# AnyDSL/rodent

Measured on AMD Instinct MI355X. Metric: Mrays/s, higher is better.
Workload: dtype f32; 1 GPU; atrium.bvh + atrium-primary.rays (1024x1024 primary rays, tmax 5000, closest hit); bvh_layout=BVH2, kernel=k_bvh2_top_auto<false,15, 255, 16, 32>, variant=top, parallelism=replicated BVH x 1, world_size=1

## Files before the change

### include/rodent_traversal.h

```cpp
#ifndef RODENT_TRAVERSAL_H
#define RODENT_TRAVERSAL_H

#include <stdint.h>
#include <stddef.h>

#ifdef __cplusplus
extern "C" {
#endif


struct Node2 {
    float   bounds[12];
    int32_t child[2];
    int32_t pad[2];
};

struct Tri1 {
    float   v0[3];  int32_t pad;
    float   e1[3];  int32_t geom_id;
    float   e2[3];  int32_t prim_id;
};

struct Node4 {
    float   bounds[6][4];
// ... 35 lines not shown
        const struct Ray1* rays, struct Hit1* hits, int32_t num_rays);
void hip_occluded_single_ray1_bvh4_tri4(int32_t dev,
        const struct Node4* nodes, const struct Tri4* tris,
        const struct Ray1* rays, struct Hit1* hits, int32_t num_rays);
void hip_intersect_single_ray1_bvh8_tri4(int32_t dev,
        const struct Node8* nodes, const struct Tri4* tris,
        const struct Ray1* rays, struct Hit1* hits, int32_t num_rays);
void hip_occluded_single_ray1_bvh8_tri4(int32_t dev,
        const struct Node8* nodes, const struct Tri4* tris,
        const struct Ray1* rays, struct Hit1* hits, int32_t num_rays);

void hip_traverse_bvh2_tri1_async(int32_t dev,
        const struct Node2* nodes, const struct Tri1* tris,
        const struct Ray1* rays, struct Hit1* hits, int32_t num_rays,
        int32_t any_hit, int32_t variant, void* stream);
void hip_traverse_bvh4_tri4_async(int32_t dev,
        const struct Node4* nodes, const struct Tri4* tris,
        const struct Ray1* rays, struct Hit1* hits, int32_t num_rays,
        int32_t any_hit, int32_t variant, void* stream);
void hip_traverse_bvh8_tri4_async(int32_t dev,
        const struct Node8* nodes, const struct Tri4* tris,
        const struct Ray1* rays, struct Hit1* hits, int32_t num_rays,
        int32_t any_hit, int32_t variant, void* stream);
int32_t rodent_hip_check_errors(int32_t dev, void* stream);

uint64_t    rodent_hip_get_kernel_time(void);
int32_t     rodent_hip_device_count(void);
int32_t     rodent_hip_num_variants(int32_t bvh_width);
void        rodent_hip_phased_min_rays(int32_t rays);
void        rodent_hip_top_min_rays(int32_t rays);
void        rodent_hip_schedule_history(int32_t enable);
void        rodent_hip_ray_kind_hint(int32_t enable);
void        rodent_hip_ray_grid(int32_t width);
int32_t     rodent_hip_is_lab_build(void);
const char* rodent_hip_variant_name(int32_t bvh_width, int32_t variant);
const char* rodent_hip_kernel_name(int32_t bvh_width, int32_t variant, int32_t any_hit);
const char* rodent_hip_version(void);
const char* rodent_hip_source_digest(void);
void        rodent_hip_read_stats(int32_t dev, uint64_t* out8);
void        rodent_hip_read_trace(int32_t dev, uint64_t* out);
void        rodent_hip_debug_set_perm(int32_t dev, const int32_t* device_perm);

#ifdef __cplusplus
}
#endif
#endif
```

### rodent_amd/abi.py

```python
from __future__ import annotations

import ctypes as C
import os
from pathlib import Path

import numpy as np
import torch

from . import formats as F

LAB = os.environ.get("RODENT_HIP_LAB", "0") not in ("", "0")
LIB_PATH = Path(__file__).resolve().parent / "lib" / ("librodent_hip_lab.so" if LAB else "librodent_hip.so")
if os.environ.get("RODENT_HIP_LIB"):
    LIB_PATH = Path(os.environ["RODENT_HIP_LIB"]).resolve()

SYNC_ENTRY_POINTS = [
    "amdgpu_intersect_single_ray1_bvh2_tri1", "amdgpu_occluded_single_ray1_bvh2_tri1",
    "hip_intersect_single_ray1_bvh4_tri4", "hip_occluded_single_ray1_bvh4_tri4",
    "hip_intersect_single_ray1_bvh8_tri4", "hip_occluded_single_ray1_bvh8_tri4",
]
ASYNC_ENTRY_POINTS = ["hip_traverse_bvh2_tri1_async", "hip_traverse_bvh4_tri4_async", "hip_traverse_bvh8_tri4_async"]
EXPORTS = SYNC_ENTRY_POINTS + ASYNC_ENTRY_POINTS + [
    "rodent_hip_check_errors", "rodent_hip_get_kernel_time", "rodent_hip_device_count", "rodent_hip_num_variants",
        "rodent_hip_variant_name",
    "rodent_hip_kernel_name", "rodent_hip_version", "rodent_hip_source_digest", "rodent_hip_is_lab_build", "rodent_hip_phased_min_rays",
        "rodent_hip_top_min_rays", "rodent_hip_ray_kind_hint", "rodent_hip_ray_grid", "rodent_hip_schedule_history",
        "rodent_hip_read_stats", "rodent_hip_read_trace", "rodent_hip_debug_set_perm",
    "rodent_hip_build_scratch_bytes", "rodent_hip_build_bvh2_tri1", "rodent_hip_build_bvh2_tri1_sync",
    "rodent_hip_build_opt_scratch_bytes", "rodent_hip_build_bvh2_tri1_opt", "rodent_hip_build_bvh2_tri1_opt_sync",
    "rodent_hip_build_split_max_refs", "rodent_hip_build_split_scratch_bytes", "rodent_hip_build_bvh2_tri1_split",
    "rodent_hip_build_bvh2_tri1_split_sync",
    "rodent_hip_refit_scratch_bytes", "rodent_hip_refit_bvh2_tri1", "rodent_hip_refit_bvh2_tri1_sync",
    "rodent_hip_refit_wide_scratch_bytes", "rodent_hip_refit_bvh4_tri4", "rodent_hip_refit_bvh4_tri4_sync",
    "rodent_hip_refit_bvh8_tri4", "rodent_hip_refit_bvh8_tri4_sync",
]
BLOCK_OF_WIDTH = {2: F.BVH2_TRI1, 4: F.BVH4_TRI4, 8: F.BVH8_TRI4}

_lib = None


class BuildOptions(C.Structure):
    _fields_ = [("max_leaf", C.c_int32), ("treelet_passes", C.c_int32), ("node_cost", C.c_float), ("tri_cost", C.c_float)]


class SplitOptions(C.Structure):
    _fields_ = [("budget", C.c_float), ("max_pieces", C.c_int32)]


class MissingExtension(RuntimeError):
    pass


def lib():
    global _lib
    if _lib is None:
        if not LIB_PATH.exists():
            raise MissingExtension(f"{LIB_PATH} not built: run `python -m rodent_amd.build` (needs hipcc)")
        l = C.CDLL(str(LIB_PATH))
        vp, i32 = C.c_void_p, C.c_int32
        for name in SYNC_ENTRY_POINTS:
            fn = getattr(l, name); fn.restype = None; fn.argtypes = [i32, vp, vp, vp, vp, i32]
        for name in ASYNC_ENTRY_POINTS:
            fn = getattr(l, name); fn.restype = None; fn.argtypes = [i32, vp, vp, vp, vp, i32, i32, i32, vp]
        l.rodent_hip_check_errors.restype = i32; l.rodent_hip_check_errors.argtypes = [i32, vp]
        l.rodent_hip_is_lab_build.restype = i32; l.rodent_hip_is_lab_build.argtypes = []
        l.rodent_hip_phased_min_rays.restype = None; l.rodent_hip_phased_min_rays.argtypes = [i32]
        l.rodent_hip_top_min_rays.restype = None; l.rodent_hip_top_min_rays.argtypes = [i32]
        l.rodent_hip_get_kernel_time.restype = C.c_uint64; l.rodent_hip_get_kernel_time.argtypes = []
        l.rodent_hip_ray_kind_hint.restype = None; l.rodent_hip_ray_kind_hint.argtypes = [i32]
        l.rodent_hip_ray_grid.restype = None; l.rodent_hip_ray_grid.argtypes = [i32]
        l.rodent_hip_schedule_history.restype = None; l.rodent_hip_schedule_history.argtypes = [i32]
        l.rodent_hip_device_count.restype = i32; l.rodent_hip_device_count.argtypes = []
        l.rodent_hip_num_variants.restype = i32; l.rodent_hip_num_variants.argtypes = [i32]
        l.rodent_hip_variant_name.restype = C.c_char_p; l.rodent_hip_variant_name.argtypes = [i32, i32]
        l.rodent_hip_kernel_name.restype = C.c_char_p; l.rodent_hip_kernel_name.argtypes = [i32, i32, i32]
        l.rodent_hip_version.restype = C.c_char_p; l.rodent_hip_version.argtypes = []
        l.rodent_hip_source_digest.restype = C.c_char_p; l.rodent_hip_source_digest.argtypes = []
        l.rodent_hip_read_trace.restype = None; l.rodent_hip_read_trace.argtypes = [i32, C.c_void_p]
        l.rodent_hip_debug_set_perm.restype = None; l.rodent_hip_debug_set_perm.argtypes = [i32, C.c_void_p]
        l.rodent_hip_read_stats.restype = None; l.rodent_hip_read_stats.argtypes = [i32, C.POINTER(C.c_uint64)]
        l.rodent_hip_build_scratch_bytes.restype = C.c_int64; l.rodent_hip_build_scratch_bytes.argtypes = [i32]
        l.rodent_hip_build_bvh2_tri1.restype = i32
        l.rodent_hip_build_bvh2_tri1.argtypes = [i32, vp, i32, vp, i32, i32, vp, vp, vp, vp, vp]
        l.rodent_hip_build_bvh2_tri1_sync.restype = i32
        l.rodent_hip_build_bvh2_tri1_sync.argtypes = [i32, vp, i32, vp, i32, i32, vp, vp, C.POINTER(i32)]
        opt = C.POINTER(BuildOptions)
        l.rodent_hip_build_opt_scratch_bytes.restype = C.c_int64; l.rodent_hip_build_opt_scratch_bytes.argtypes = [i32, opt]
        l.rodent_hip_build_bvh2_tri1_opt.restype = i32
        l.rodent_hip_build_bvh2_tri1_opt.argtypes = [i32, vp, i32, vp, i32, opt, vp, vp, vp, vp, vp]
        l.rodent_hip_build_bvh2_tri1_opt_sync.restype = i32
        l.rodent_hip_build_bvh2_tri1_opt_sync.argtypes = [i32, vp, i32, vp, i32, opt, vp, vp, C.POINTER(i32)]
        spl = C.POINTER(SplitOptions)
        l.rodent_hip_build_split_max_refs.restype = C.c_int64; l.rodent_hip_build_split_max_refs.argtypes = [i32, spl]
        l.rodent_hip_build_split_scratch_bytes.restype = C.c_int64
        l.rodent_hip_build_split_scratch_bytes.argtypes = [i32, opt, spl]
        l.rodent_hip_build_bvh2_tri1_split.restype = i32
        l.rodent_hip_build_bvh2_tri1_split.argtypes = [i32, vp, i32, vp, i32, opt, spl, vp, vp, vp, vp, vp]
        l.rodent_hip_build_bvh2_tri1_split_sync.restype = i32
        l.rodent_hip_build_bvh2_tri1_split_sync.argtypes = [i32, vp, i32, vp, i32, opt, spl, vp, vp, C.POINTER(i32)]
        l.rodent_hip_refit_scratch_bytes.restype = C.c_int64; l.rodent_hip_refit_scratch_bytes.argtypes = [i32, i32]
        l.rodent_hip_refit_bvh2_tri1.restype = i32
        l.rodent_hip_refit_bvh2_tri1.argtypes = [i32, vp, i32, vp, i32, vp, i32, vp, i32, vp, vp, vp]
        l.rodent_hip_refit_bvh2_tri1_sync.restype = i32
# ... 84 lines not shown
    n = len(rays)
    rays_dev = to_device(rays, bvh.dev)
    hits_dev = torch.zeros(max(n, 1) * F.HIT1.itemsize, dtype=torch.uint8, device=f"cuda:{bvh.dev}")
    if variant is None:
        torch.cuda.synchronize(bvh.dev)
        name = {(2, False): "amdgpu_intersect_single_ray1_bvh2_tri1", (2, True): "amdgpu_occluded_single_ray1_bvh2_tri1",
                (4, False): "hip_intersect_single_ray1_bvh4_tri4", (4, True): "hip_occluded_single_ray1_bvh4_tri4",
                (8, False): "hip_intersect_single_ray1_bvh8_tri4",
                    (8, True): "hip_occluded_single_ray1_bvh8_tri4"}[(bvh.width, bool(any_hit))]
        getattr(lib(), name)(bvh.dev, bvh.nodes.data_ptr(), bvh.tris.data_ptr(), rays_dev.data_ptr(), hits_dev.data_ptr(), n)
    else:
        traverse_async(bvh, rays_dev, hits_dev, n, any_hit, variant)
        torch.cuda.synchronize(bvh.dev)
        check_errors(bvh.dev)
    return from_device(hits_dev, F.HIT1)[:n]


def schedule_history(enable: bool):
    lib().rodent_hip_schedule_history(int(bool(enable)))


def top_min_rays(rays: int):
    lib().rodent_hip_top_min_rays(int(rays))


def ray_kind_hint(enable: bool):
    lib().rodent_hip_ray_kind_hint(int(bool(enable)))


def ray_grid(width: int = -1):
    lib().rodent_hip_ray_grid(int(width))


def check_errors(dev=0, stream=None):
    import torch
    if stream is None:
        stream = torch.cuda.current_stream(dev)
    if lib().rodent_hip_check_errors(dev, C.c_void_p(stream.cuda_stream)):
        raise RuntimeError("rodent_hip: traversal stack overflow (more than 64 entries)")


def read_stats(dev=0):
    buf = (C.c_uint64 * 8)()
    lib().rodent_hip_read_stats(dev, buf)
    return list(buf)


def read_trace(dev=0, arm_only=False):
    if arm_only:
        lib().rodent_hip_read_trace(dev, None)
        return None
    buf = np.zeros((16384, 4), np.uint64)
    lib().rodent_hip_read_trace(dev, buf.ctypes.data_as(C.c_void_p))
    return buf
```

### rodent_amd/csrc/traversal.hip

```cpp
#include <hip/hip_runtime.h>

#include <algorithm>
#include <atomic>
#include <cstdint>
#include <cstdio>
#include <cstdlib>
#include <memory>
#include <mutex>
#include <utility>
#include <vector>

#include "device_buffer.h"
#include "rodent_traversal.h"
#include "traversal_device.h"

namespace {

using namespace rodent_dev;

template <bool ANY, bool WIDE = true>
__device__ __forceinline__ bool leaf_tri1(const Tri1* __restrict__ tris, int first, RayX& ray, HitAcc& hit) {
    int j = first;
    for (;;) {
        const float4* p = WIDE ? reinterpret_cast<const float4*>(tris + j)
// ... 83 lines not shown
        if (last) {
            ctl->stats[7] += (unsigned long long)count; ctl->counter = 0; ctl->deep_count = 0; ctl->finish_done = 0;
            report_error(ctl);
        }
    }
}

template <bool ANY>
__global__ __launch_bounds__(kWave) void k_bvh2_finish(const Node2* __restrict__ nodes, const Tri1* __restrict__ tris,
                                                        const Ray1* __restrict__ rays, Hit1* __restrict__ hits,
                                                        Ctl* ctl, const int* __restrict__ deep_list,
                                                            int* , int* phase_counters) {
    __shared__ int stack_lds[kStackCap * kWave];
    finish_launch<ANY>(nodes, tris, rays, hits, ctl, deep_list, (lds_int*)stack_lds, phase_counters, blockIdx.x, gridDim.x);
}

struct Lane {
    RayX ray;
    int top;
    lds_int* sp;
    int ray_id;
    bool found;
};
typedef const __attribute__((address_space(1))) char* gptr;
struct Bases { gptr node, tri; };
__device__ __forceinline__ Bases make_bases(const Node2* nodes, const Tri1* tris) {
    unsigned long long node_bits = reinterpret_cast<unsigned long long>(nodes - 1), tri_bits = reinterpret_cast<unsigned long long>(tris);
    asm volatile("" : "+v"(node_bits), "+v"(tri_bits));
    return Bases{(gptr)node_bits, (gptr)tri_bits};
}

typedef __attribute__((address_space(3))) float lds_float;
template <bool ANY, bool PF = false, bool TOP = false, bool LAZY = false, bool FENCE = false, bool SHARED = false, int SPILL = 0,
    int WPG = 1>
__device__ __forceinline__ void bvh2_step(Lane& L, const Bases& base, Hit1* __restrict__ hits, lds_int* sp_limit, Ctl* ctl,
    int* __restrict__ deep_list,
                                          bool prefetch = false, lds_int* pf_row = nullptr, lds_int* image = nullptr,
                                              lds_float* shared_tmax = nullptr,
                                          int* __restrict__ spill = nullptr) {
    const bool is_node = L.top > 0;
    typedef float f32x4 __attribute__((ext_vector_type(4)));
    typedef int i32x2 __attribute__((ext_vector_type(2)));
    f32x4 q0, q1, q2;
    i32x2 ch;
    int popped;
    float shared_now = 0.0f;
    if constexpr (TOP && !SHARED) {
        const unsigned idx = (unsigned)(is_node ? L.top : ~L.top), stride = is_node ? (unsigned)sizeof(Node2) : (unsigned)sizeof(Tri1);
        const gptr addr = (is_node ? base.node : base.tri) + (size_t)idx * stride;
        joint_fetch(q0, q1, q2, ch, popped, L.top >= kLdsTag, (unsigned)(size_t)image + (unsigned)(L.top - kLdsTag), addr,
            addr + (is_node ? 48u : 40u), L.sp);
    } else {
        if (TOP && L.top >= kLdsTag) {
            typedef __attribute__((address_space(3))) const char* lds_bytes;
            const lds_bytes rec = (lds_bytes)image + (unsigned)(L.top - kLdsTag);
            const __attribute__((address_space(3))) f32x4* p = (const __attribute__((address_space(3))) f32x4*)rec;
            q0 = p[0]; q1 = p[1]; q2 = p[2];
            ch = *(const __attribute__((address_space(3))) i32x2*)(rec + 48);
        } else {
            const unsigned idx = (unsigned)(is_node ? L.top : ~L.top), stride = is_node ? (unsigned)sizeof(Node2) : (unsigned)sizeof(Tri1);
            const gptr addr = (is_node ? base.node : base.tri) + (size_t)idx * stride;
            const __attribute__((address_space(1))) f32x4* p = (const __attribute__((address_space(1))) f32x4*)addr;
            q0 = p[0]; q1 = p[1]; q2 = p[2];
            ch = *(const __attribute__((address_space(1))) i32x2*)(addr + (is_node ? 48u : 40u));
        }
        popped = *L.sp;
        if (SHARED) shared_now = *shared_tmax;
        asm volatile("" : "+v"(q0), "+v"(q1), "+v"(q2), "+v"(ch));
    }
    if (SHARED) {
        L.ray.tmax = shared_now;
        if (ANY && shared_now == -__builtin_inff()) { L.top = 0; return; }
    }
    if (PF && prefetch && is_node) {
#pragma unroll
        for (int k = 0; k < 2; k++) {
            const int c = k ? ch.y : ch.x;
            const bool inner = c > 0;
            const gptr a = (inner ? base.node : base.tri) + (size_t)(unsigned)(inner ? c : ~c) * (inner ? (unsigned)sizeof(Node2)
                : (unsigned)sizeof(Tri1));
            if (c != 0) __builtin_amdgcn_global_load_lds((const __attribute__((address_space(1))) void*)a,
                (__attribute__((address_space(3))) void*)pf_row, 4, 0, 0);
        }
    }
    if (is_node) {
        float te0, te1;
        const bool h0 = slab_canonical(L.ray, q0.x, q0.y, q0.z, q0.w, q1.x, q1.y, te0) && ch.x != 0;
        const bool h1 = slab_canonical(L.ray, q1.z, q1.w, q2.x, q2.y, q2.z, q2.w, te1) && ch.y != 0;
        const bool c0first = te0 < te1, both = h0 && h1;
        L.sp[kWave] = c0first ? ch.y : ch.x;
        L.top = both ? (c0first ? ch.x : ch.y) : (h0 ? ch.x : (h1 ? ch.y : popped));
        L.sp += (both ? kWave : 0) - ((h0 || h1) ? 0 : kWave);
        if (both && L.sp >= sp_limit) {
            if constexpr (SPILL > 0) stack_spill<SPILL>(L.sp, L.top, sp_limit, spill, WPG, &ctl->err, &ctl->stats[7]);
            else {
                deep_list[atomicAdd(&ctl->deep_count, 1)] = L.ray_id;
                L.top = 0;
                if (LAZY) L.found = true;
                if (FENCE) __threadfence();
            }
        }
    } else {
        const int prim_id = __float_as_int(q2.w);
        const float nx = cross_x(q1.x, q1.y, q1.z, q2.x, q2.y, q2.z);
        const float ny = cross_y(q1.x, q1.y, q1.z, q2.x, q2.y, q2.z);
        const float nz = cross_z(q1.x, q1.y, q1.z, q2.x, q2.y, q2.z);
        float t, u, v;
        bool found = false;
        if (intersect_tri(L.ray, q0.x, q0.y, q0.z, q1.x, q1.y, q1.z, q2.x, q2.y, q2.z, nx, ny, nz, t, u, v)) {
            if (SHARED) {
                __builtin_amdgcn_ds_fminf(shared_tmax, ANY ? -__builtin_inff() : t, 0, 0, false);
                if (ANY || *shared_tmax == t) store_hit(hits, L.ray_id, prim_id & 0x7FFFFFFF, t, u, v);
            } else store_hit(hits, L.ray_id, prim_id & 0x7FFFFFFF, t, u, v);
            L.ray.tmax = t; found = true;
            if (LAZY) L.found = true;
        }
        const bool leave = prim_id < 0;
        L.top = (ANY && found) ? 0 : (leave ? popped : L.top - 1);
        L.sp -= (leave && !(ANY && found)) ? kWave : 0;
    }
    if constexpr (SPILL > 0) if (L.top >= kSpillMark) stack_reload<SPILL>(L.sp, L.top, sp_limit, spill, WPG);
// ... 392 lines not shown
constexpr int kSpillSlots = 9216;
void ensure_spill(DeviceState& s, int slots) {
    int want = 64;
    while (want < slots) want *= 2;
    s.spill.ensure((size_t)std::min(want, kSpillSlots) * kSpillWaveInts);
}
int persistent_groups(const DeviceState& s, int occ, int waves) {
    const int groups = ((s.num_cus * (occ / waves) + kStripes - 1) / kStripes) * kStripes;
    if ((long)groups * waves > kSpillSlots) {
        fprintf(stderr, "rodent_hip: %d x %d resident waves exceed the %d stack spill blocks\n", groups, waves, kSpillSlots); abort(); }
    return groups;
}

bool read_and_clear_error_flags(DeviceState& s, hipStream_t stream) {
    HIP_CHECK(hipStreamSynchronize(stream));
    volatile int* page = s.host_page;
    const bool raised = page[kHostErr] != 0;
    page[kHostErr] = 0;
    return raised;
}
void check_error_flag(DeviceState& s, hipStream_t stream) {
    if (read_and_clear_error_flags(s, stream)) {
        fprintf(stderr, "rodent_hip: traversal stack overflow (more than %d entries)\n", kStackCap); abort(); }
}

int mapped_node_ids(const Node2* nodes) {
    hipDeviceptr_t range_base = nullptr; size_t range_size = 0;
    if (hipMemGetAddressRange(&range_base, &range_size, (hipDeviceptr_t)nodes) != hipSuccess) { (void)hipGetLastError(); return 0; }
    const size_t bytes = (size_t)((const char*)range_base + range_size - (const char*)nodes);
    return (int)std::min<size_t>(bytes / sizeof(Node2), 0x3FFFFFFF);
}

int g_ray_grid = [] { const char* e = getenv("RODENT_HIP_RAY_GRID"); return e ? atoi(e) : -1; }();
int g_schedule_history = [] { const char* e = getenv("RODENT_HIP_SCHEDULE_HISTORY"); return e && atoi(e) ? 1 : 0; }();
constexpr int kFinishGroups = 256;
#define LAUNCH_ARGS DeviceState& s, const Node2* nodes, const Tri1* tris, const Ray1* rays, Hit1* hits, int n, hipStream_t stream

constexpr int kGridMinRays = 2048 * kWave;
bool reserve_single(DeviceState& s, int n, bool spill) {
    s.deep_list.ensure(n);
    spill = spill && blocks_for(n) <= kSpillSlots;
    if (spill) ensure_spill(s, blocks_for(n));
    return spill;
}
template <bool ANY, int LDS_N, int XCD, bool TR = false, int PRIO = 0> void L_single(LAUNCH_ARGS) {
    if (reserve_single(s, n, PRIO == 0 && !TR))
        hipLaunchKernelGGL((k_bvh2_single<ANY, LDS_N, XCD, false, 0, true>), dim3(blocks_for(n)), dim3(kWave), 0, stream, nodes, tris,
            rays, hits, n, s.ctl(), s.deep_list.ptr, (const int*)nullptr, s.spill.ptr, n >= kGridMinRays ? g_ray_grid : 0);
    else
        hipLaunchKernelGGL((k_bvh2_single<ANY, LDS_N, XCD, TR, PRIO>), dim3(blocks_for(n)), dim3(kWave), 0, stream, nodes, tris, rays,
            hits, n, s.ctl(), s.deep_list.ptr, (const int*)nullptr, (int*)nullptr, 0);
    hipLaunchKernelGGL((k_bvh2_finish<ANY>), dim3(kFinishGroups), dim3(kWave), 0, stream, nodes, tris, rays, hits, s.ctl(),
        s.deep_list.ptr, s.deep_stack, (int*)nullptr);
}


template <bool ANY, int LDS_N, int TOPN, int WAVES, bool PREFETCH, bool SORTED, int OCC, bool TRACE = false, int PRIO = 0, int FUSED = 0,
    bool LAZY = false> void launch_top_persist(LAUNCH_ARGS, int max_id) {
    const int groups = persistent_groups(s, OCC, WAVES);
    s.deep_list.ensure(n);
    ensure_spill(s, groups * WAVES);
    ensure_top_buffers(s);
    s.top_image_nodes = nullptr;
    const int* perm = nullptr;
    if (SORTED) {
        ensure_sort_buffers(s, n);
// ... 47 lines not shown
    const int max_id = top_kernel_ids(nodes, n);
    if (max_id == 0) { reserve_single(s, n, true); return 0; }
    const int groups = persistent_groups(s, 32, waves);
    s.deep_list.ensure(n);
    ensure_top_buffers(s);
    ensure_spill(s, groups * waves);
    if (g_schedule_history && stripe_chunks(n) <= kMaxStripeChunks) ensure_history(s);
    return max_id;
}
template <bool ANY, int LDS_N, int TOPN, int WAVES, int REFILL, int MODE = 0, bool FUSED = true,
    bool LAZY = false> void L_default(LAUNCH_ARGS) {
    const int max_id = reserve_default(s, nodes, n, WAVES);
    if (max_id == 0) { L_single<ANY, 16, 32>(s, nodes, tris, rays, hits, n, stream); return; }
    if (g_schedule_history) {
        launch_top_persist<ANY, LDS_N, TOPN, WAVES, false, false, 32, false, 0, 2>(s, nodes, tris, rays, hits, n, stream, max_id); return; }
    const int groups = persistent_groups(s, 32, WAVES);
    s.top_image_nodes = nullptr; s.order_rays = 0;
    if (s.hint_rays != rays || s.hint_n != n) { s.hint_rays = rays; s.hint_n = n; s.hint_first_id = s.launch_id + 1; }
    const int id = ++s.launch_id;
    const volatile int* kinds = s.host_kinds;
    const bool hinting = MODE == 0 && g_kind_hint;
    int* const report_to = hinting ? s.host_kinds : nullptr;
    const bool incoherent = hinting && kinds[1] >= s.hint_first_id && kinds[0] < kinds[1];
    if (incoherent) {
        hipLaunchKernelGGL((k_bvh2_top_refill<ANY, LDS_N, TOPN, WAVES, REFILL, false, false>), dim3(groups), dim3(kWave * WAVES), 0,
            stream, nodes, tris, rays, hits, n, s.ctl(), s.deep_list.ptr,
                           (const int4*)s.top_image.ptr, s.tickets.ptr, max_id, s.spill.ptr, report_to, id);
        hipLaunchKernelGGL((k_bvh2_top_finish<ANY>), dim3(1), dim3(kWave), 0, stream, nodes, tris, rays, hits, s.ctl(), s.deep_list.ptr,
            s.deep_stack, s.tickets.ptr, s.top_image.ptr, TOPN);
        return;
    }
    hipLaunchKernelGGL((k_bvh2_top_auto<ANY, LDS_N, TOPN, WAVES, REFILL, MODE, FUSED, LAZY>), dim3(groups), dim3(kWave * WAVES), 0, stream,
        nodes, tris, rays, hits, n, s.ctl(), s.deep_list.ptr,
                       s.top_image.ptr, s.tickets.ptr, max_id, s.spill.ptr, report_to, id, g_ray_grid);
    if (!FUSED) hipLaunchKernelGGL((k_bvh2_top_finish<ANY>), dim3(1), dim3(kWave), 0, stream, nodes, tris, rays, hits, s.ctl(),
        s.deep_list.ptr, s.deep_stack, s.tickets.ptr, s.top_image.ptr, TOPN);
}

template <bool ANY, int LDS_N, int TOPN, int WAVES, int REFILL, bool ADAPT = false, bool FENCE = false> void L_top_refill(LAUNCH_ARGS) {
    if (top_kernel_ids(nodes, n) == 0) { L_single<ANY, 16, 32>(s, nodes, tris, rays, hits, n, stream); return; }
    const int groups = persistent_groups(s, 32, WAVES);
    s.deep_list.ensure(n);
    ensure_top_buffers(s);
    s.top_image_nodes = nullptr;
    ensure_spill(s, groups * WAVES);
    hipLaunchKernelGGL((k_bvh2_top_refill<ANY, LDS_N, TOPN, WAVES, REFILL, ADAPT, FENCE>), dim3(groups), dim3(kWave * WAVES), 0, stream,
        nodes, tris, rays, hits, n, s.ctl(), s.deep_list.ptr,
                       (const int4*)s.top_image.ptr, s.tickets.ptr, mapped_node_ids(nodes), s.spill.ptr, (int*)nullptr, 0);
    hipLaunchKernelGGL((k_bvh2_top_finish<ANY>), dim3(1), dim3(kWave), 0, stream, nodes, tris, rays, hits, s.ctl(), s.deep_list.ptr,
        s.deep_stack, s.tickets.ptr, s.top_image.ptr, TOPN);
}



template <bool ANY, int LDS_N> void L_sorted(LAUNCH_ARGS) {
    s.deep_list.ensure(n);
    ensure_sort_buffers(s, n);
    const int blocks = (n + kSortBlockRays - 1) / kSortBlockRays;
    hipLaunchKernelGGL(k_raysort_count, dim3(blocks), dim3(kSortThreads), 0, stream, nodes, rays, n, s.sort_keys.ptr, s.sort_totals.ptr);
    hipLaunchKernelGGL(k_raysort_scan, dim3(1), dim3(kSortCells), 0, stream, s.sort_totals.ptr, s.sort_totals.ptr + kSortCells);
    hipLaunchKernelGGL(k_raysort_scatter, dim3(blocks), dim3(kSortThreads), 0, stream, s.sort_keys.ptr, n, s.sort_totals.ptr + kSortCells,
        s.sort_perm.ptr);
    hipLaunchKernelGGL((k_bvh2_single<ANY, LDS_N, 32, false, 0>), dim3(blocks_for(n)), dim3(kWave), 0, stream, nodes, tris, rays, hits, n,
        s.ctl(), s.deep_list.ptr, (const int*)s.sort_perm.ptr, (int*)nullptr, 0);
    hipLaunchKernelGGL((k_bvh2_finish<ANY>), dim3(kFinishGroups), dim3(kWave), 0, stream, nodes, tris, rays, hits, s.ctl(),
        s.deep_list.ptr, s.deep_stack, (int*)nullptr);
}
// ... 185 lines not shown
    timed_sync_call(dev, num_rays, nullptr,
        [&](DeviceState& s) { launch_wide(8, false, s, nodes, tris, rays, hits, num_rays, default_variant(8), nullptr); });
}
void hip_occluded_single_ray1_bvh8_tri4(int32_t dev, const Node8* nodes, const Tri4* tris, const Ray1* rays, Hit1* hits, int32_t num_rays) {
    timed_sync_call(dev, num_rays, nullptr,
        [&](DeviceState& s) { launch_wide(8, true, s, nodes, tris, rays, hits, num_rays, default_variant(8), nullptr); });
}

int32_t rodent_hip_device_count(void) {
    int count = 0;
    if (hipGetDeviceCount(&count) != hipSuccess) return 0;
    return count;
}
int32_t rodent_hip_num_variants(int32_t bvh_width) {
    if (bvh_width == 2) return kNumVariants2;
    int count = 0; wide_variants(bvh_width, &count); return count;
}
const char* rodent_hip_variant_name(int32_t bvh_width, int32_t variant) {
    if (bvh_width == 2) return variant >= 0 && variant < kNumVariants2 ? kVariants2[variant].name : "";
    int count = 0; const VariantW* t = wide_variants(bvh_width, &count);
    return variant >= 0 && variant < count ? t[variant].name : "";
}
const char* rodent_hip_kernel_name(int32_t bvh_width, int32_t variant, int32_t any_hit) {
    if (bvh_width == 2) return variant >= 0 && variant < kNumVariants2 ? kVariants2[variant].kernel[any_hit ? 1 : 0] : "";
    int count = 0; const VariantW* t = wide_variants(bvh_width, &count);
    return variant >= 0 && variant < count ? t[variant].kernel[any_hit ? 1 : 0] : "";
}
void rodent_hip_phased_min_rays(int32_t rays) { g_phased_min_rays = rays < 0 ? 4096 * kWave : rays; }
void rodent_hip_debug_set_perm(int32_t dev, const int32_t* device_perm) { device_state(dev).debug_perm = device_perm; }
void rodent_hip_schedule_history(int32_t enable) { g_schedule_history = enable ? 1 : 0; }
void rodent_hip_top_min_rays(int32_t rays) { g_top_min_rays = rays < 0 ? kTopMinRays : rays; }
void rodent_hip_ray_kind_hint(int32_t enable) { g_kind_hint = enable ? 1 : 0; }
void rodent_hip_ray_grid(int32_t width) { g_ray_grid = width; }
int32_t rodent_hip_is_lab_build(void) {
#ifdef RODENT_HIP_LAB
    return 1;
#else
    return 0;
#endif
}
void rodent_hip_read_trace(int32_t dev, uint64_t* out) {
    DeviceState& s = device_state(dev);
    HIP_CHECK(hipSetDevice(dev));
    HIP_CHECK(hipDeviceSynchronize());
    std::lock_guard<std::mutex> launching(s.mutex);
    const size_t bytes = 16384 * 4 * sizeof(uint64_t);
    if (!s.trace.ptr) {
        s.trace.ensure(16384 * 4, 0);
        HIP_CHECK(hipMemcpy(&s.ctl()->trace, &s.trace.ptr, sizeof(void*), hipMemcpyHostToDevice));
    }
    if (out) HIP_CHECK(hipMemcpy(out, s.trace.ptr, bytes, hipMemcpyDeviceToHost));
    HIP_CHECK(hipMemset(s.trace.ptr, 0, bytes));
}
void rodent_hip_read_stats(int32_t dev, uint64_t* out) {
    DeviceState& s = device_state(dev);
    HIP_CHECK(hipSetDevice(dev));
    HIP_CHECK(hipDeviceSynchronize());
    HIP_CHECK(hipMemcpy(out, s.ctl()->stats, 8 * sizeof(uint64_t), hipMemcpyDeviceToHost));
    HIP_CHECK(hipMemset(s.ctl()->stats, 0, 8 * sizeof(uint64_t)));
}
const char* rodent_hip_version(void) { return "rodent_hip 0.2 (gfx950)"; }

}
```

### rodent_amd/csrc/traversal_device.h

```cpp
#pragma once
#include <hip/hip_runtime.h>
#include <cstdint>
#include "rodent_traversal.h"

namespace rodent_dev {

constexpr int   kWave = 64;
constexpr int   kStackCap = 64;
constexpr float kFltMax = 3.4028234664e+38f;

struct RayX {
    float ox, oy, oz, dx, dy, dz, idx, idy, idz, iox, ioy, ioz, tmin, tmax;
};

__device__ __forceinline__ float prodsign(float x, float y) {
    return __int_as_float(__float_as_int(x) ^ (__float_as_int(y) & (int)0x80000000u));
}
__device__ __forceinline__ float safe_rcp(float x) {
    return (fabsf(x) < 1e-8f) ? prodsign(kFltMax, x) : 1.0f / x;
}
__device__ __forceinline__ float dot3(float ax, float ay, float az, float bx, float by, float bz) {
    return fmaf(az, bz, fmaf(ay, by, ax * bx));
}
__device__ __forceinline__ float cross_x(float ax, float ay, float az, float bx, float by, float bz) { return fmaf(ay, bz, -(az * by)); }
__device__ __forceinline__ float cross_y(float ax, float ay, float az, float bx, float by, float bz) { return fmaf(az, bx, -(ax * bz)); }
__device__ __forceinline__ float cross_z(float ax, float ay, float az, float bx, float by, float bz) { return fmaf(ax, by, -(ay * bx)); }

__device__ __forceinline__ RayX load_ray(const Ray1* rays, int i) {
    const float4* p = reinterpret_cast<const float4*>(rays + i);
    const float4 r0 = p[0], r1 = p[1];
    RayX r;
    r.ox = r0.x; r.oy = r0.y; r.oz = r0.z; r.tmin = r0.w;
    r.dx = r1.x; r.dy = r1.y; r.dz = r1.z; r.tmax = r1.w;
    r.idx = safe_rcp(r.dx); r.idy = safe_rcp(r.dy); r.idz = safe_rcp(r.dz);
    r.iox = -(r.ox * r.idx); r.ioy = -(r.oy * r.idy); r.ioz = -(r.oz * r.idz);
    return r;
}

__device__ __forceinline__ void store_hit(Hit1* hits, int i, int id, float t, float u, float v) {
    *reinterpret_cast<float4*>(hits + i) = make_float4(__int_as_float(id), t, u, v);
}

typedef float f32x2 __attribute__((ext_vector_type(2)));
__device__ __forceinline__ bool slab(const RayX& r, float lox, float hix, float loy, float hiy, float loz, float hiz, float& tentry) {
    const f32x2 tx = __builtin_elementwise_fma((f32x2){r.idx, r.idx}, (f32x2){lox, hix}, (f32x2){r.iox, r.iox});
    const f32x2 ty = __builtin_elementwise_fma((f32x2){r.idy, r.idy}, (f32x2){loy, hiy}, (f32x2){r.ioy, r.ioy});
    const f32x2 tz = __builtin_elementwise_fma((f32x2){r.idz, r.idz}, (f32x2){loz, hiz}, (f32x2){r.ioz, r.ioz});
    tentry = fmaxf(fmaxf(fminf(tx.x, tx.y), fminf(ty.x, ty.y)), fmaxf(fminf(tz.x, tz.y), r.tmin));
    const float texit = fminf(fminf(fmaxf(tx.x, tx.y), fmaxf(ty.x, ty.y)), fminf(fmaxf(tz.x, tz.y), r.tmax));
    return tentry <= texit;
}

__device__ __forceinline__ float canonical(float x) { return __builtin_canonicalizef(x); }
__device__ __forceinline__ bool slab_canonical(const RayX& r, float lox, float hix, float loy, float hiy, float loz, float hiz,
    float& tentry) {
    const f32x2 tx = __builtin_elementwise_fma((f32x2){r.idx, r.idx}, (f32x2){lox, hix}, (f32x2){r.iox, r.iox});
    const f32x2 ty = __builtin_elementwise_fma((f32x2){r.idy, r.idy}, (f32x2){loy, hiy}, (f32x2){r.ioy, r.ioy});
    const f32x2 tz = __builtin_elementwise_fma((f32x2){r.idz, r.idz}, (f32x2){loz, hiz}, (f32x2){r.ioz, r.ioz});
    float nz, fz;
    asm("v_max_f32 %0, %1, %2" : "=v"(nz) : "v"(fminf(tz.x, tz.y)), "v"(r.tmin));
    asm("v_min_f32 %0, %1, %2" : "=v"(fz) : "v"(fmaxf(tz.x, tz.y)), "v"(r.tmax));
    tentry = fmaxf(fmaxf(fminf(tx.x, tx.y), fminf(ty.x, ty.y)), nz);
    const float texit = fminf(fminf(fmaxf(tx.x, tx.y), fmaxf(ty.x, ty.y)), fz);
    return tentry <= texit;
}

__device__ __forceinline__ bool intersect_tri(const RayX& r,
                                              float v0x, float v0y, float v0z, float e1x, float e1y, float e1z,
                                              float e2x, float e2y, float e2z, float nx, float ny, float nz,
                                              float& t_out, float& u_out, float& v_out) {
    const float cx = v0x - r.ox, cy = v0y - r.oy, cz = v0z - r.oz;
    const float rx = cross_x(r.dx, r.dy, r.dz, cx, cy, cz);
    const float ry = cross_y(r.dx, r.dy, r.dz, cx, cy, cz);
    const float rz = cross_z(r.dx, r.dy, r.dz, cx, cy, cz);
    const float det = dot3(nx, ny, nz, r.dx, r.dy, r.dz);
    const float abs_det = fabsf(det);
    const float u = prodsign(dot3(rx, ry, rz, e2x, e2y, e2z), det);
    const float v = prodsign(dot3(rx, ry, rz, e1x, e1y, e1z), det);
    if (!(u >= 0.0f) || !(v >= 0.0f) || !(u + v <= abs_det)) return false;
    const float t = prodsign(dot3(cx, cy, cz, nx, ny, nz), det);
    if (!(abs_det != 0.0f)) return false;
    if (!(t >= abs_det * r.tmin) || !(t <= abs_det * r.tmax)) return false;
    const float inv_det = 1.0f / abs_det;
    t_out = t * inv_det; u_out = u * inv_det; v_out = v * inv_det;
    return true;
}


struct HitAcc { int id; float t, u, v; };

typedef __attribute__((address_space(3))) int lds_int;

constexpr int kLdsTag = 0x40000000;

constexpr int kSpillMark = 0x7F000000;
constexpr int kSpillRows = 7, kSpillBlocks = 7;
constexpr int kSpillWaveInts = kSpillRows * kSpillBlocks * kWave;
// ... 102 lines not shown
```

### rodent_amd/csrc/traversal_top.h

```cpp
#pragma once

template <int TOPN>
__global__ __launch_bounds__(kWave) void k_bvh2_top_image(const Node2* __restrict__ nodes, int4* __restrict__ image) {
    __shared__ int slot_node[TOPN];
    build_top_image(nodes, image, TOPN, (lds_int*)slot_node);
}

template <bool ANY>
__global__ __launch_bounds__(kWave) void k_bvh2_top_finish(const Node2* __restrict__ nodes, const Tri1* __restrict__ tris,
                                                            const Ray1* __restrict__ rays, Hit1* __restrict__ hits,
                                                            Ctl* ctl, const int* __restrict__ deep_list, int* deep_stack, int* tickets,
                                                            int4* __restrict__ image, int capacity) {
    __shared__ int stack_lds[kStackCap * kWave];
    static_assert(kStackCap * kWave >= kMaxTopNodes, "slot table");
    const bool stale = ctl->reserved != 0;
    finish_launch<ANY>(nodes, tris, rays, hits, ctl, deep_list, (lds_int*)stack_lds, tickets, blockIdx.x, gridDim.x);
    if (stale && blockIdx.x == 0) {
        build_top_image(nodes, image, capacity, (lds_int*)stack_lds);
        if (threadIdx.x == 0) ctl->reserved = 0;
    }
}


__device__ __forceinline__ int stripe_rank(int wave) { return wave * ((int)gridDim.x / kStripes) + (int)blockIdx.x / kStripes; }
// ... 262 lines not shown
            const int want = kWave - __popcll(live);
            int first = 0;
            if (lane == 0) first = atomicAdd(counter, want);
            first = stripe_waves * kWave + __builtin_amdgcn_readfirstlane(first);
            more = ray_of(first) < n;
            if (L.top == 0) {
                const int r = ray_of(first + __popcll(~live & ((1ull << lane) - 1ull)));
                if (r < n) {
                    L = start_lane(rays, hits, r, r, col);
                    L.top = root;
                }
            }
            if (ADAPT) need = one_origin(__ballot(L.top != 0) & ~live) ? kWave : REFILL;
            continue;
        }
        if (live == 0) break;
        if (L.top != 0) bvh2_step<ANY, false, true, false, false, false, LDS_N, WAVES>(L, base, hits, sp_limit, ctl, deep_list, false,
            nullptr, image, nullptr, spill);
    }
}

template <bool ANY, int LDS_N, int TOPN, int WAVES, int REFILL, bool ADAPT = false, bool FENCE = false>
__global__ __launch_bounds__(kWave * WAVES, 32 / WAVES) void k_bvh2_top_refill(const Node2* __restrict__ nodes,
    const Tri1* __restrict__ tris,
                                                                    const Ray1* __restrict__ rays, Hit1* __restrict__ hits, int n,
                                                                    Ctl* ctl, int* __restrict__ deep_list,
                                                                        const int4* __restrict__ top_image, int* __restrict__ tickets,
                                                                        int max_id,
                                                                    int* spill, int* host_kinds, int launch_id) {
    top_refill_body<ANY, LDS_N, TOPN, WAVES, REFILL, ADAPT, FENCE>(nodes, tris, rays, hits, n, ctl, deep_list, top_image, tickets, max_id,
        spill, host_kinds, launch_id);
}

template <bool ANY, int LDS_N, int TOPN, int WAVES, int REFILL,
    int MODE = 0 ,
    bool FUSED = true , bool LAZY = false>
__global__ __launch_bounds__(kWave * WAVES) __attribute__((amdgpu_waves_per_eu(8, 8))) void
    k_bvh2_top_auto(const Node2* __restrict__ nodes, const Tri1* __restrict__ tris,
                                                                  const Ray1* __restrict__ rays, Hit1* __restrict__ hits, int n,
                                                                  Ctl* ctl, int* __restrict__ deep_list, int4* __restrict__ top_image,
                                                                      int* __restrict__ tickets, int max_id,
                                                                  int* spill, int* host_kinds, int launch_id, int grid_w) {
    constexpr int kStackInts = WAVES * (LDS_N + 1) * kWave, kGroupRays = 32 * kWave;
    static_assert((kStackInts + TOPN * 16) * 4 * (32 / WAVES) <= 160 * 1024, "32 waves per CU must fit their stacks and images in LDS");
    __shared__ __attribute__((aligned(16))) int lds_raw[kStackInts + TOPN * 16];
    const int lane = threadIdx.x % kWave, wave = threadIdx.x / kWave;
    lds_int* col = (lds_int*)lds_raw + wave * (LDS_N + 1) * kWave + lane;
    lds_int* image = (lds_int*)lds_raw + kStackInts;
    const int root = stage_top_image<TOPN, kWave * WAVES>(nodes, (const int4*)top_image, image, (lds_int*)lds_raw, ctl, max_id)
        ? kLdsTag : 1;
    if (root != 1 && threadIdx.x == 0 && blockIdx.x == 0) atomicAdd(&ctl->stats[6], 1ull);
    const int stripe = blockIdx.x % kStripes, stripe_waves = (gridDim.x / kStripes) * WAVES;
    int* counter = tickets + stripe * kCounterStride;
    const auto ray_of = [&](int t) { return ((t / kGroupRays) * kStripes + stripe) * kGroupRays + t % kGroupRays; };
    lds_int* const sp_limit = col + LDS_N * kWave;
    const Bases base = make_bases(nodes, tris);
    int t = stripe_rank(wave) * kWave;
    bool coherent = MODE != 2;
    if (MODE == 0 && ray_of(t) < n) {
        const int r = ray_of(t + lane);
        const float4* p = reinterpret_cast<const float4*>(rays + (r < n ? r : ray_of(t)));
        const float4 o = p[0], d = p[1];
        if (grid_w < 0) grid_w = detect_ray_grid(rays, n);
        coherent = wave_rays_coherent(o.x, o.y, o.z, d.x, d.y, d.z, r < n);
        if (wave == 0) report_ray_kind(host_kinds, launch_id, coherent);
    }
    if (!coherent && threadIdx.x == 0 && blockIdx.x == 0) atomicAdd(&ctl->stats[5], 1ull);
    grid_w = __builtin_amdgcn_readfirstlane(grid_w > 0 && (grid_w & 7) == 0 ? grid_w : 0);
    const int tiled_rays = tiled_ray_count(grid_w, n);
    if (grid_w > 0 && threadIdx.x == 0 && blockIdx.x == 0) atomicAdd(&ctl->stats[2], (unsigned long long)grid_w);
    if (MODE == 1 || (MODE == 0 && coherent)) {
        for (;;) {
            int first_ray = ray_of(t);
            if (first_ray >= n) break;
            int r = ray_of(t + lane);
            if (first_ray < tiled_rays) r = tile_ray(first_ray, lane, grid_w);
            Lane L = start_lane<LAZY>(rays, hits, r < n ? r : -1, first_ray, col);
            if (L.top != 0) L.top = root;
            while (__ballot(L.top != 0)) {
                if (L.top != 0) bvh2_step<ANY, false, true, LAZY, false, false, LDS_N, WAVES>(L, base, hits, sp_limit, ctl, deep_list,
                    false, nullptr, image, nullptr, spill);
            }
            if (LAZY) finish_lane_reg(L, rays, hits);
            int t_next = 0;
            if (lane == 0) t_next = atomicAdd(counter, kWave);
            t = stripe_waves * kWave + __builtin_amdgcn_readfirstlane(t_next);
        }
    } else if (MODE != 1) {
        const auto ray_at = [&](int pos) { return pos < tiled_rays ? tile_ray_at(pos, grid_w) : pos; };
        Lane L;
        {
            const int r = ray_at(ray_of(t + lane));
            L = start_lane<LAZY>(rays, hits, r < n ? r : -1, 0, col);
            if (L.top != 0) L.top = root;
        }
        bool more = true;
        for (;;) {
            const unsigned long long live = __ballot(L.top != 0);
            if (more && __popcll(live) <= kWave - REFILL) {
                const int want = kWave - __popcll(live);
                int first = 0;
                if (lane == 0) first = atomicAdd(counter, want);
                first = stripe_waves * kWave + __builtin_amdgcn_readfirstlane(first);
                more = ray_of(first) < n;
                if (L.top == 0) {
                    if (LAZY) { finish_lane_reg(L, rays, hits); L.ray_id = -1; }
                    const int pos = ray_of(first + __popcll(~live & ((1ull << lane) - 1ull)));
                    if (pos < n) {
                        const int rr = ray_at(pos);
                        L = start_lane<LAZY>(rays, hits, rr, rr, col);
                        L.top = root;
                    }
                }
                continue;
            }
// ... 23 lines not shown
```

Baseline: 5992 Mrays/s.

## Specialize BVH2 top traversal loops per wave-uniform ray octant

Adds eight octant-specialized copies of the coherent traversal loop. A wave whose active rays all share one direction octant and have finite values uses a version where the near and far slab planes are picked at compile time, which removes the per-axis min/max in the box test. Ray inverse-direction splats are precomputed once per chunk, and the hit pointer is pre-offset by the ray id so the per-step ray id is zero. The cost is a much larger kernel body, with more instruction-cache and register pressure. It also relies on the assumption that a lane's hit index does not depend on L.ray_id elsewhere, and the stack start now comes from window_base instead of col.

```diff
diff --git a/include/rodent_traversal.h b/include/rodent_traversal.h
--- a/include/rodent_traversal.h
+++ b/include/rodent_traversal.h
@@ -91,6 +91,7 @@
 void        rodent_hip_schedule_history(int32_t enable);
 void        rodent_hip_ray_kind_hint(int32_t enable);
 void        rodent_hip_ray_grid(int32_t width);
+void        rodent_hip_octant_loops(int32_t enable);
 int32_t     rodent_hip_is_lab_build(void);
 const char* rodent_hip_variant_name(int32_t bvh_width, int32_t variant);
 const char* rodent_hip_kernel_name(int32_t bvh_width, int32_t variant, int32_t any_hit);
diff --git a/rodent_amd/abi.py b/rodent_amd/abi.py
--- a/rodent_amd/abi.py
+++ b/rodent_amd/abi.py
@@ -24,7 +24,7 @@
     "rodent_hip_check_errors", "rodent_hip_get_kernel_time", "rodent_hip_device_count", "rodent_hip_num_variants",
         "rodent_hip_variant_name",
     "rodent_hip_kernel_name", "rodent_hip_version", "rodent_hip_source_digest", "rodent_hip_is_lab_build", "rodent_hip_phased_min_rays",
-        "rodent_hip_top_min_rays", "rodent_hip_ray_kind_hint", "rodent_hip_ray_grid", "rodent_hip_schedule_history",
+        "rodent_hip_top_min_rays", "rodent_hip_ray_kind_hint", "rodent_hip_ray_grid", "rodent_hip_octant_loops", "rodent_hip_schedule_history",
         "rodent_hip_read_stats", "rodent_hip_read_trace", "rodent_hip_debug_set_perm",
     "rodent_hip_build_scratch_bytes", "rodent_hip_build_bvh2_tri1", "rodent_hip_build_bvh2_tri1_sync",
     "rodent_hip_build_opt_scratch_bytes", "rodent_hip_build_bvh2_tri1_opt", "rodent_hip_build_bvh2_tri1_opt_sync",
@@ -69,6 +69,7 @@
         l.rodent_hip_get_kernel_time.restype = C.c_uint64; l.rodent_hip_get_kernel_time.argtypes = []
         l.rodent_hip_ray_kind_hint.restype = None; l.rodent_hip_ray_kind_hint.argtypes = [i32]
         l.rodent_hip_ray_grid.restype = None; l.rodent_hip_ray_grid.argtypes = [i32]
+        l.rodent_hip_octant_loops.restype = None; l.rodent_hip_octant_loops.argtypes = [i32]
         l.rodent_hip_schedule_history.restype = None; l.rodent_hip_schedule_history.argtypes = [i32]
         l.rodent_hip_device_count.restype = i32; l.rodent_hip_device_count.argtypes = []
         l.rodent_hip_num_variants.restype = i32; l.rodent_hip_num_variants.argtypes = [i32]
@@ -219,6 +220,10 @@
     lib().rodent_hip_ray_grid(int(width))
 
 
+def octant_loops(enable: bool = True):
+    lib().rodent_hip_octant_loops(int(bool(enable)))
+
+
 def check_errors(dev=0, stream=None):
     import torch
     if stream is None:
diff --git a/rodent_amd/csrc/traversal.hip b/rodent_amd/csrc/traversal.hip
--- a/rodent_amd/csrc/traversal.hip
+++ b/rodent_amd/csrc/traversal.hip
@@ -139,12 +139,12 @@
 
 typedef __attribute__((address_space(3))) float lds_float;
 template <bool ANY, bool PF = false, bool TOP = false, bool LAZY = false, bool FENCE = false, bool SHARED = false, int SPILL = 0,
-    int WPG = 1>
+    int WPG = 1, int OCT = -1>
 __device__ __forceinline__ void bvh2_step(Lane& L, const Bases& base, Hit1* __restrict__ hits, lds_int* sp_limit, Ctl* ctl,
     int* __restrict__ deep_list,
                                           bool prefetch = false, lds_int* pf_row = nullptr, lds_int* image = nullptr,
                                               lds_float* shared_tmax = nullptr,
-                                          int* __restrict__ spill = nullptr) {
+                                          int* __restrict__ spill = nullptr, const RaySplat* splat = nullptr) {
     const bool is_node = L.top > 0;
     typedef float f32x4 __attribute__((ext_vector_type(4)));
     typedef int i32x2 __attribute__((ext_vector_type(2)));
@@ -192,8 +192,8 @@
     }
     if (is_node) {
         float te0, te1;
-        const bool h0 = slab_canonical(L.ray, q0.x, q0.y, q0.z, q0.w, q1.x, q1.y, te0) && ch.x != 0;
-        const bool h1 = slab_canonical(L.ray, q1.z, q1.w, q2.x, q2.y, q2.z, q2.w, te1) && ch.y != 0;
+        const bool h0 = slab_canonical<OCT>(L.ray, q0.x, q0.y, q0.z, q0.w, q1.x, q1.y, te0, splat) && ch.x != 0;
+        const bool h1 = slab_canonical<OCT>(L.ray, q1.z, q1.w, q2.x, q2.y, q2.z, q2.w, te1, splat) && ch.y != 0;
         const bool c0first = te0 < te1, both = h0 && h1;
         L.sp[kWave] = c0first ? ch.y : ch.x;
         L.top = both ? (c0first ? ch.x : ch.y) : (h0 ? ch.x : (h1 ? ch.y : popped));
@@ -652,6 +652,7 @@
 }
 
 int g_ray_grid = [] { const char* e = getenv("RODENT_HIP_RAY_GRID"); return e ? atoi(e) : -1; }();
+int g_octant_loops = [] { const char* e = getenv("RODENT_HIP_OCTANT_LOOPS"); return e ? (atoi(e) ? 1 : 0) : 1; }();
 int g_schedule_history = [] { const char* e = getenv("RODENT_HIP_SCHEDULE_HISTORY"); return e && atoi(e) ? 1 : 0; }();
 constexpr int kFinishGroups = 256;
 #define LAUNCH_ARGS DeviceState& s, const Node2* nodes, const Tri1* tris, const Ray1* rays, Hit1* hits, int n, hipStream_t stream
@@ -765,7 +766,7 @@
     }
     hipLaunchKernelGGL((k_bvh2_top_auto<ANY, LDS_N, TOPN, WAVES, REFILL, MODE, FUSED, LAZY>), dim3(groups), dim3(kWave * WAVES), 0, stream,
         nodes, tris, rays, hits, n, s.ctl(), s.deep_list.ptr,
-                       s.top_image.ptr, s.tickets.ptr, max_id, s.spill.ptr, report_to, id, g_ray_grid);
+                       s.top_image.ptr, s.tickets.ptr, max_id, s.spill.ptr, report_to, id, g_ray_grid, g_octant_loops);
     if (!FUSED) hipLaunchKernelGGL((k_bvh2_top_finish<ANY>), dim3(1), dim3(kWave), 0, stream, nodes, tris, rays, hits, s.ctl(),
         s.deep_list.ptr, s.deep_stack, s.tickets.ptr, s.top_image.ptr, TOPN);
 }
@@ -1017,6 +1018,7 @@
 void rodent_hip_top_min_rays(int32_t rays) { g_top_min_rays = rays < 0 ? kTopMinRays : rays; }
 void rodent_hip_ray_kind_hint(int32_t enable) { g_kind_hint = enable ? 1 : 0; }
 void rodent_hip_ray_grid(int32_t width) { g_ray_grid = width; }
+void rodent_hip_octant_loops(int32_t enable) { g_octant_loops = enable ? 1 : 0; }
 int32_t rodent_hip_is_lab_build(void) {
 #ifdef RODENT_HIP_LAB
     return 1;
diff --git a/rodent_amd/csrc/traversal_device.h b/rodent_amd/csrc/traversal_device.h
--- a/rodent_amd/csrc/traversal_device.h
+++ b/rodent_amd/csrc/traversal_device.h
@@ -52,17 +52,45 @@
 }
 
 __device__ __forceinline__ float canonical(float x) { return __builtin_canonicalizef(x); }
+struct RaySplat { f32x2 idx, idy, idz, iox, ioy, ioz; };
+constexpr int kAnyOctant = -1, kAnyOctantSplat = -2;
+__device__ __forceinline__ RaySplat splat_ray(const RayX& r) {
+    RaySplat s{(f32x2){r.idx, r.idx}, (f32x2){r.idy, r.idy}, (f32x2){r.idz, r.idz}, (f32x2){r.iox, r.iox}, (f32x2){r.ioy, r.ioy},
+        (f32x2){r.ioz, r.ioz}};
+    asm volatile("" : "+v"(s.idx), "+v"(s.idy), "+v"(s.idz), "+v"(s.iox), "+v"(s.ioy), "+v"(s.ioz));
+    return s;
+}
+template <int OCT = -1>
 __device__ __forceinline__ bool slab_canonical(const RayX& r, float lox, float hix, float loy, float hiy, float loz, float hiz,
-    float& tentry) {
-    const f32x2 tx = __builtin_elementwise_fma((f32x2){r.idx, r.idx}, (f32x2){lox, hix}, (f32x2){r.iox, r.iox});
-    const f32x2 ty = __builtin_elementwise_fma((f32x2){r.idy, r.idy}, (f32x2){loy, hiy}, (f32x2){r.ioy, r.ioy});
-    const f32x2 tz = __builtin_elementwise_fma((f32x2){r.idz, r.idz}, (f32x2){loz, hiz}, (f32x2){r.ioz, r.ioz});
-    float nz, fz;
-    asm("v_max_f32 %0, %1, %2" : "=v"(nz) : "v"(fminf(tz.x, tz.y)), "v"(r.tmin));
-    asm("v_min_f32 %0, %1, %2" : "=v"(fz) : "v"(fmaxf(tz.x, tz.y)), "v"(r.tmax));
-    tentry = fmaxf(fmaxf(fminf(tx.x, tx.y), fminf(ty.x, ty.y)), nz);
-    const float texit = fminf(fminf(fmaxf(tx.x, tx.y), fmaxf(ty.x, ty.y)), fz);
-    return tentry <= texit;
+    float& tentry, const RaySplat* splat = nullptr) {
+    if constexpr (OCT < 0) {
+        const bool pairs = OCT == kAnyOctantSplat;
+        const f32x2 tx = pairs ? __builtin_elementwise_fma(splat->idx, (f32x2){lox, hix}, splat->iox)
+            : __builtin_elementwise_fma((f32x2){r.idx, r.idx}, (f32x2){lox, hix}, (f32x2){r.iox, r.iox});
+        const f32x2 ty = pairs ? __builtin_elementwise_fma(splat->idy, (f32x2){loy, hiy}, splat->ioy)
+            : __builtin_elementwise_fma((f32x2){r.idy, r.idy}, (f32x2){loy, hiy}, (f32x2){r.ioy, r.ioy});
+        const f32x2 tz = pairs ? __builtin_elementwise_fma(splat->idz, (f32x2){loz, hiz}, splat->ioz)
+            : __builtin_elementwise_fma((f32x2){r.idz, r.idz}, (f32x2){loz, hiz}, (f32x2){r.ioz, r.ioz});
+        float nz, fz;
+        asm("v_max_f32 %0, %1, %2" : "=v"(nz) : "v"(fminf(tz.x, tz.y)), "v"(r.tmin));
+        asm("v_min_f32 %0, %1, %2" : "=v"(fz) : "v"(fmaxf(tz.x, tz.y)), "v"(r.tmax));
+        tentry = fmaxf(fmaxf(fminf(tx.x, tx.y), fminf(ty.x, ty.y)), nz);
+        const float texit = fminf(fminf(fmaxf(tx.x, tx.y), fmaxf(ty.x, ty.y)), fz);
+        return tentry <= texit;
+    } else {
+        const f32x2 tx = __builtin_elementwise_fma(splat->idx, (f32x2){lox, hix}, splat->iox);
+        const f32x2 ty = __builtin_elementwise_fma(splat->idy, (f32x2){loy, hiy}, splat->ioy);
+        const f32x2 tz = __builtin_elementwise_fma(splat->idz, (f32x2){loz, hiz}, splat->ioz);
+        const float nearx = (OCT & 1) ? tx.y : tx.x, farx = (OCT & 1) ? tx.x : tx.y;
+        const float neary = (OCT & 2) ? ty.y : ty.x, fary = (OCT & 2) ? ty.x : ty.y;
+        const float nearz = (OCT & 4) ? tz.y : tz.x, farz = (OCT & 4) ? tz.x : tz.y;
+        float nz, fz;
+        asm("v_max_f32 %0, %1, %2" : "=v"(nz) : "v"(nearz), "v"(r.tmin));
+        asm("v_min_f32 %0, %1, %2" : "=v"(fz) : "v"(farz), "v"(r.tmax));
+        tentry = fmaxf(fmaxf(nearx, neary), nz);
+        const float texit = fminf(fminf(farx, fary), fz);
+        return tentry <= texit;
+    }
 }
 
 __device__ __forceinline__ bool intersect_tri(const RayX& r,
diff --git a/rodent_amd/csrc/traversal_top.h b/rodent_amd/csrc/traversal_top.h
--- a/rodent_amd/csrc/traversal_top.h
+++ b/rodent_amd/csrc/traversal_top.h
@@ -318,6 +318,25 @@
         spill, host_kinds, launch_id);
 }
 
+__device__ __forceinline__ int chunk_octant(const Lane& L) {
+    const RayX& r = L.ray;
+    const auto negative = [](float x) { return (int)((unsigned)__float_as_int(x) >> 31); };
+    const int oct = negative(r.idx) | (negative(r.idy) << 1) | (negative(r.idz) << 2);
+    const auto finite3 = [](float x, float y, float z) { return __builtin_isfinite(x) && __builtin_isfinite(y) && __builtin_isfinite(z); };
+    const bool finite = finite3(r.ox, r.oy, r.oz) && finite3(r.dx, r.dy, r.dz) && finite3(r.idx, r.idy, r.idz)
+        && finite3(r.iox, r.ioy, r.ioz);
+    const int first = __builtin_amdgcn_readfirstlane(oct);
+    return __ballot(L.ray_id >= 0 && !(finite && oct == first)) == 0ull ? first : -1;
+}
+template <bool ANY, bool LAZY, int LDS_N, int WAVES, int OCT>
+__device__ __forceinline__ void trace_chunk(Lane& L, const Bases& base, Hit1* __restrict__ hits, lds_int* sp_limit, Ctl* ctl,
+    int* __restrict__ deep_list, lds_int* image, int* __restrict__ spill, const RaySplat* splat) {
+    while (__ballot(L.top != 0)) {
+        if (L.top != 0) bvh2_step<ANY, false, true, LAZY, false, false, LDS_N, WAVES, OCT>(L, base, hits, sp_limit, ctl, deep_list,
+            false, nullptr, image, nullptr, spill, splat);
+    }
+}
+
 template <bool ANY, int LDS_N, int TOPN, int WAVES, int REFILL,
     int MODE = 0 ,
     bool FUSED = true , bool LAZY = false>
@@ -326,7 +345,8 @@
                                                                   const Ray1* __restrict__ rays, Hit1* __restrict__ hits, int n,
                                                                   Ctl* ctl, int* __restrict__ deep_list, int4* __restrict__ top_image,
                                                                       int* __restrict__ tickets, int max_id,
-                                                                  int* spill, int* host_kinds, int launch_id, int grid_w) {
+                                                                  int* spill, int* host_kinds, int launch_id, int grid_w,
+                                                                      int octant_loops) {
     constexpr int kStackInts = WAVES * (LDS_N + 1) * kWave, kGroupRays = 32 * kWave;
     static_assert((kStackInts + TOPN * 16) * 4 * (32 / WAVES) <= 160 * 1024, "32 waves per CU must fit their stacks and images in LDS");
     __shared__ __attribute__((aligned(16))) int lds_raw[kStackInts + TOPN * 16];
@@ -361,12 +381,25 @@
             if (first_ray >= n) break;
             int r = ray_of(t + lane);
             if (first_ray < tiled_rays) r = tile_ray(first_ray, lane, grid_w);
-            Lane L = start_lane<LAZY>(rays, hits, r < n ? r : -1, first_ray, col);
+            Lane L = start_lane<LAZY>(rays, hits, r < n ? r : -1, first_ray, window_base<LDS_N>(sp_limit));
             if (L.top != 0) L.top = root;
-            while (__ballot(L.top != 0)) {
-                if (L.top != 0) bvh2_step<ANY, false, true, LAZY, false, false, LDS_N, WAVES>(L, base, hits, sp_limit, ctl, deep_list,
-                    false, nullptr, image, nullptr, spill);
-            }
+            const int oct = octant_loops ? chunk_octant(L) : -1;
+            if (oct >= 0 && lane == 0 && blockIdx.x == 0) atomicAdd(&ctl->stats[3], 1ull);
+            int arm = oct;
+            const RaySplat splat = splat_ray(L.ray);
+            static_assert(LDS_N > 0, "bvh2_step<SPILL = LDS_N>: the ray id is only the hit record's index");
+            const int ray_id = L.ray_id;
+            Hit1* lane_hit = hits + ray_id;
+            asm volatile("" : "+v"(lane_hit));
+            L.ray_id = 0;
+#define RODENT_TRACE_CHUNK(OCT) if (arm == OCT) trace_chunk<ANY, LAZY, LDS_N, WAVES, OCT>(L, base, lane_hit, sp_limit, ctl, deep_list, image, spill, \
+                &splat); \
+            asm volatile("" : "+s"(arm))
+            RODENT_TRACE_CHUNK(0); RODENT_TRACE_CHUNK(1); RODENT_TRACE_CHUNK(2); RODENT_TRACE_CHUNK(3);
+            RODENT_TRACE_CHUNK(4); RODENT_TRACE_CHUNK(5); RODENT_TRACE_CHUNK(6); RODENT_TRACE_CHUNK(7);
+#undef RODENT_TRACE_CHUNK
+            trace_chunk<ANY, LAZY, LDS_N, WAVES, kAnyOctantSplat>(L, base, lane_hit, sp_limit, ctl, deep_list, image, spill, &splat);
+            L.ray_id = ray_id;
             if (LAZY) finish_lane_reg(L, rays, hits);
             int t_next = 0;
             if (lane == 0) t_next = atomicAdd(counter, kWave);
```

After: 6404 Mrays/s (median of 6 runs). 1.07x the previous value.
